# ChristophReich1996/Multi-StyleGAN

Measured on AMD Instinct MI355X. Metric: training images/sec (G+D step, 256^2, seq=3x2ch), higher is better.
Workload: dtype bf16

## Files before the change

multi_stylegan_amd/csrc/conv_wgrad.hip:

```cpp
#include "msg_common.h"
#include <stdlib.h>

typedef __bf16 bf16v8 __attribute__((ext_vector_type(8)));
typedef short s16x4 __attribute__((ext_vector_type(4)));
typedef const __attribute__((address_space(1))) char* gptr_t;
typedef const __attribute__((address_space(1))) u32x4* gvec_t;
typedef __attribute__((address_space(3))) char* lds_t;
__device__ __attribute__((aligned(256))) unsigned int g_wgrad_zero_page[64];

struct WgradParams {
    int B, IH, IW, Cx, I, OH, OW, ldgy, O;
    int OWv, OHv;
    int kh, kw, stride, pad, pixel_shuffle;
    int per_sample, chunks_per_sample, pix_per_chunk, split;
    int xcd_slices;
    int nz;
    int fold;
    int o_tiles, i_tiles, ldgw;
    int oi_major;
    float gain;
    long long gw_zstride;
    long long slab;
};

// ... 392 lines not shown
    float4 t = part[0][lane];
#pragma unroll
    for (int g = 1; g < 4; ++g) { t.x += part[g][lane].x; t.y += part[g][lane].y; t.z += part[g][lane].z; t.w += part[g][lane].w; }
    if (!oi_major) {
        reinterpret_cast<float4*>(out + (long long)n * slab)[v] = t;
        return;
    }
    const int vpr = ldgw >> 2;
    const long long row = v / vpr;
    const int i = (int)(v - row * vpr) * 4;
    const int o = (int)(row / taps), tap = (int)(row - (long long)o * taps);
    float* dst = out + ((long long)n * O + o) * I * taps + (long long)i * taps + tap;
    const float e[4] = {t.x, t.y, t.z, t.w};
#pragma unroll
    for (int k = 0; k < 4; ++k)
        if (i + k < I) dst[(long long)k * taps] = e[k];
}

extern "C" int msg_wgrad_reduce_launch(const float* ws, float* gw, long long slab, int n_out, int chunks, int O, int taps,
                                       int I, int ldgw, int oi_major, void* stream) {
    const long long nvec = slab >> 2;
    const long long blocks = (nvec + 63) / 64;
    if (blocks >= (1ll << 31) || n_out > 65535) return MSG_EUNSUPPORTED;
    hipLaunchKernelGGL(wgrad_reduce_kernel, dim3((unsigned)blocks, (unsigned)n_out), dim3(256), 0, (hipStream_t)stream,
                       ws, gw, slab, chunks, O, taps, I, ldgw, oi_major);
    return MSG_CHECK_LAUNCH();
}

extern "C" int msg_conv2d_wgrad_row3_try(const void* gy, const void* x, float* gw, int dtype,
                                         int B, int IH, int IW, int Cx, int I, int OH, int OW, int ldgy, int O, int ldgw,
                                         int kh, int kw, int stride, int pad, int pixel_shuffle,
                                         int per_sample, int k_chunks, int oi_major, float gain,
                                         float* ws, long long ws_floats, int plan_only, long long* need, void* stream);

static int wgrad_impl(const void* gy, const void* x, float* gw, int dtype,
                      int B, int IH, int IW, int Cx, int I, int OH, int OW, int ldgy, int O, int ldgw,
                      int kh, int kw, int stride, int pad, int pixel_shuffle,
                      int per_sample, int k_chunks, int oi_major, float gain,
                      float* ws, long long ws_floats, int plan_only, long long* need, void* stream) {
    *need = 0;
    if (B == 0) return MSG_OK;
    if (B < 0 || IH <= 0 || IW <= 0 || OH <= 0 || OW <= 0 || O <= 0 || I <= 0 || kh <= 0 ||
        kw <= 0 || stride <= 0 || Cx <= 0 || ldgy <= 0 || ldgw < I || ldgw % 4 || k_chunks <= 0)
        return MSG_EINVAL;
    if (!plan_only && (!gy || !x || !gw)) return MSG_EINVAL;
    const int split = dtype == MSG_F32_SPLIT ? 3 : 0;
    if (split) dtype = MSG_F32;
    if (dtype != MSG_F32 && dtype != MSG_BF16) return MSG_EUNSUPPORTED;
    const int esz = dtype == MSG_BF16 ? 2 : 4, vec = 16 / esz;
    if (Cx % vec || ldgy % vec) return MSG_EUNSUPPORTED;
    if (!plan_only && (((uintptr_t)gy | (uintptr_t)x | (uintptr_t)gw | (uintptr_t)ws) & 15u)) return MSG_EUNSUPPORTED;
    {
        const int r3 = msg_conv2d_wgrad_row3_try(gy, x, gw, dtype, B, IH, IW, Cx, I, OH, OW, ldgy, O, ldgw, kh, kw, stride, pad,
                                                 pixel_shuffle, per_sample, k_chunks, oi_major, gain, ws, ws_floats, plan_only,
                                                 need, stream);
        if (r3 < 0) return r3;
        if (r3) return MSG_OK;
    }
    WgradParams p{};
    p.B = B; p.IH = IH; p.IW = IW; p.Cx = Cx; p.I = I; p.OH = OH; p.OW = OW; p.ldgy = ldgy; p.O = O;
    p.kh = kh; p.kw = kw; p.stride = stride; p.pad = pad; p.pixel_shuffle = pixel_shuffle;
    p.per_sample = per_sample;
    p.chunks_per_sample = k_chunks;
    const int kp = dtype == MSG_BF16 ? 64 : 32;
    static const int variant = msg_tunable("MSG_CONV_VARIANT", 0);
    static const int pad_rows = msg_tunable("MSG_WGRAD_PAD_ROWS", 1);
    const long long gy_bytes = (long long)(pixel_shuffle ? 4 : 1) * OH * OW * ldgy * esz;
    const long long x_bytes = (long long)IH * IW * Cx * esz;
    int owv = OW, ohv = OH;
    if (pad_rows && !pixel_shuffle && !(kp % OW == 0 || OW % kp == 0)) {
        int v = 1;
        while (v < OW) v <<= 1;
        if ((long long)v * 15 <= (long long)OW * 16) {
            owv = v;
            if (v < kp && (OH * v) % kp) ohv = ((OH * v + kp - 1) / kp * kp) / v;
        }
    }
    const bool can_fold0 = !per_sample && variant != 3;
    auto uni_ok = [&](int wl) {
        const long long np = (long long)(wl == OW ? OH : ohv) * wl;
        bool u = variant != 2 && variant != 1 && (kp % wl == 0 || wl % kp == 0) && gy_bytes < (1ll << 31) && x_bytes < (1ll << 31);
        if (can_fold0 && B * np < (1ll << 31) && u &&
            !((np % kp == 0 || kp % np == 0) && B * gy_bytes < 0x7ffffff0ll && B * x_bytes < 0x7ffffff0ll))
            u = false;
        return u;
    };
    bool uni = uni_ok(owv);
    if (!uni && owv != OW) { owv = OW; uni = uni_ok(OW); }
    if (owv == OW) ohv = OH;
    p.OWv = owv;
// ... 93 lines not shown
```

include/msg_hip.h:

```cpp
#ifndef MSG_HIP_H
#define MSG_HIP_H

#ifdef __cplusplus
extern "C" {
#endif

enum { MSG_OK = 0, MSG_EINVAL = -1, MSG_EUNSUPPORTED = -2, MSG_ELAUNCH = -3 };
enum { MSG_F32 = 0, MSG_BF16 = 1, MSG_F16 = 2, MSG_F64 = 3, MSG_F32_SPLIT = 4 };

#define MSG_ABI_VERSION 5
int msg_abi_version(void);
const char* msg_build_arch(void);
const char* msg_strerror(int code);

int msg_upfirdn2d(const void* x, const float* fir, void* y, int dtype,
                  int major, int in_h, int in_w, int minor, int kh, int kw,
                  int up_x, int up_y, int down_x, int down_y,
                  int pad_x0, int pad_x1, int pad_y0, int pad_y1, void* stream);

int msg_upfirdn2d_pitched(const void* x, const float* fir, void* y, int dtype,
                          int major, int in_h, int in_w, int minor, int in_pitch, int kh, int kw,
                          int up_x, int up_y, int down_x, int down_y,
                          int pad_x0, int pad_x1, int pad_y0, int pad_y1, void* stream);

// ... 147 lines not shown
                                  int kh, int kw, int stride, int pad, long long w_batch_stride,
                                  const void* residual, int res_ld,
                                  const unsigned char* sign_mask, int mask_tile_m, int mask_tile_n,
                                  const void* sign_map, int sign_ld, float alpha, float scale,
                                  float* grad_bias, const float* noise, int noise_batch, float* grad_noise_weight,
                                  float* ws, long long ws_floats, void* stream);

int msg_act_pointwise_head(const void* x, const float* bias, const float* w, float* y, int dtype,
                           long long npix, int C, float wscale, float alpha, float scale, void* stream);
long long msg_act_pointwise_head_backward_workspace(long long npix, int C);
int msg_act_pointwise_head_backward(const void* x, const float* bias, const float* w, const float* gy, void* gx,
                                    float* grad_bias_and_w, int dtype, long long npix, int C, float wscale,
                                    float alpha, float scale, float* ws, long long ws_floats, void* stream);

int msg_linear_fprop(const float* x, const float* w, const float* bias, float* y, int M, int N, int K,
                     float gain, float bias_gain, void* stream);
int msg_linear_dgrad(const float* gy, const float* w, float* gx, int M, int N, int K, float gain, void* stream);
int msg_linear_wgrad(const float* gy, const float* x, float* gw, float* gb, int M, int N, int K,
                     float gain, float bias_gain, void* stream);

int msg_linear_grouped_fprop(const float* x, const int* slot, const float* const* w, const float* const* bias, float* y,
                             int G, int M, int N, int K, int L, float gain, float bias_gain, void* stream);
int msg_linear_grouped_dgrad(const float* gy, const float* const* w, float* gx, int G, int M, int N, int K, float gain,
                             void* stream);
int msg_linear_grouped_wgrad(const float* gy, const float* x, const int* slot, float* gw, float* gb, int G, int M, int N,
                             int K, int L, float gain, float bias_gain, void* stream);
int msg_linear_grouped_wgrad_ptrs(const float* gy, const float* x, const int* slot, float* const* gw, float* const* gb, int G,
                                  int M, int N, int K, int L, float gain, float bias_gain, void* stream);

int msg_conv2d_fprop_plan(int dtype, int B, int IH, int IW, int Cx, int Ck, int OH, int OW, int N,
                          int kh, int kw, long long w_batch_stride);
int msg_conv2d_fprop_upconv_eligible(int B, int IH, int IW, int Cx, int Ck, int OH, int OW, int N, int kh, int kw,
                                     int stride, int pad, int in_up, int pixel_shuffle, long long w_batch_stride);
int msg_conv2d_fprop_thin_eligible(int B, int IH, int IW, int Cx, int Ck, int OH, int OW, int N, int ldy, int kh, int kw,
                                   int stride, int pad, int in_up, int pixel_shuffle, int act_mode);

int msg_flat_adam(float* param, const float* grad, float* exp_avg, float* exp_avg_sq, float* ema, long long n,
                  const float* coef, float lr, float beta1, float beta2, float eps, int step, float ema_decay,
                  void* stream);
int msg_flat_ema(float* ema, const float* param, long long n, float decay, void* stream);

#ifdef __cplusplus
}
#endif
#endif
```

multi_stylegan_amd/_lib.py:

```python
import ctypes
import os
import re

import torch

_HERE = os.path.dirname(os.path.abspath(__file__))
LIB_PATH = os.path.join(_HERE, "libmsg_hip" + ("_" + os.environ["MSG_LIB_VARIANT"] if os.environ.get("MSG_LIB_VARIANT") else "")
                        + ".so")
HEADER_PATH = os.path.join(os.path.dirname(_HERE), "include", "msg_hip.h")

MSG_F32, MSG_BF16, MSG_F16, MSG_F64 = 0, 1, 2, 3
ABI_VERSION = 5
_c = ctypes
_P, _I, _L, _F = _c.c_void_p, _c.c_int, _c.c_longlong, _c.c_float

_SIGNATURES = {
    "msg_abi_version": (_I, []),
    "msg_build_arch": (_c.c_char_p, []),
    "msg_strerror": (_c.c_char_p, [_I]),
    "msg_upfirdn2d": (_I, [_P, _P, _P, _I] + [_I] * 14 + [_P]),
    "msg_upfirdn2d_pitched": (_I, [_P, _P, _P, _I] + [_I] * 15 + [_P]),
    "msg_upfirdn2d_pitched2": (_I, [_P, _P, _P, _I] + [_I] * 16 + [_P]),
    "msg_upfirdn2d_separable": (_I, [_P, _P, _P, _P, _I] + [_I] * 10 + [_P]),
    "msg_upfirdn2d_separable_act": (_I, [_P, _P, _P, _P, _I] + [_I] * 10 + [_P, _P, _P, _I, _F, _F, _P]),
# ... 19 lines not shown
    "msg_conv2d_wgrad": (_I, [_P, _P, _P, _I] + [_I] * 18 + [_F, _P, _L, _P]),
    "msg_conv2d_wgrad_workspace": (_L, [_I] * 18),
    "msg_demod_coeff": (_I, [_P, _P, _P, _I, _I, _I, _I, _F, _F, _P]),
    "msg_scale_rows_cols": (_I, [_P, _P, _P, _P, _I, _I, _I, _I, _I, _I, _F, _P]),
    "msg_modulate_weights": (_I, [_P] * 5 + [_I] * 7 + [_F, _F, _P]),
    "msg_modulate_backward": (_I, [_P] * 6 + [_I] * 6 + [_F, _P]),
    "msg_modulate_backward2": (_I, [_P] * 7 + [_I] * 6 + [_F, _P]),
    "msg_scale_rows_cols2": (_I, [_P] * 6 + [_I] * 6 + [_F, _P]),
    "msg_relayout_weight": (_I, [_P, _P, _P, _P, _I] + [_I] * 7 + [_F, _P]),
    "msg_gather_taps": (_I, [_P, _P, _I] + [_I] * 9 + [_P]),
    "msg_fold_taps": (_I, [_P, _P, _P, _I] + [_I] * 10 + [_P]),
    "msg_scaled_add": (_I, [_P, _P, _P, _I, _L, _F, _F, _P]),
    "msg_rgb_skip_merge": (_I, [_P, _I, _I, _P, _P, _P, _P, _I, _I, _I, _I, _P]),
    "msg_rgb_skip_merge_backward": (_I, [_P, _P, _I, _I, _P, _P, _I, _I, _I, _I, _P]),
    "msg_gamma_merge": (_I, [_P, _P, _P, _P, _I, _L, _F, _P]),
    "msg_gamma_merge_backward_workspace": (_L, []),
    "msg_gamma_merge_backward": (_I, [_P, _P, _P, _P, _P, _P, _I, _L, _F, _P, _P]),
    "msg_scaled_add_rows": (_I, [_P, _P, _P, _I, _L, _I, _L, _L, _L, _F, _F, _P]),
    "msg_flat_adam": (_I, [_P, _P, _P, _P, _P, _L, _P, _F, _F, _F, _F, _I, _F, _P]),
    "msg_flat_ema": (_I, [_P, _P, _L, _F, _P]),
    "msg_softmax_rows": (_I, [_P, _P, _I, _L, _I, _P]),
    "msg_softmax_rows_backward": (_I, [_P, _P, _P, _I, _L, _I, _P]),
    "msg_softmax_rows_backward2": (_I, [_P, _P, _P, _P, _P, _I, _L, _I, _P]),
    "msg_nonlocal_attention_supported": (_I, [_I] * 5),
    "msg_nonlocal_attention_fwd": (_I, [_P] * 5 + [_I] * 6 + [_P]),
    "msg_nonlocal_attention_bwd_splits": (_I, [_I] * 3),
    "msg_nonlocal_attention_bwd": (_I, [_P] * 14 + [_I] * 6 + [_P]),
    "msg_affine_warp": (_I, [_P, _P, _P, _F, _P, _P, _P, _I, _F, _F, _I, _I, _I, _I, _I, _I, _I, _P, _P]),
    "msg_minibatch_stddev_workspace": (_L, [_I] * 5),
    "msg_minibatch_stddev": (_I, [_P, _P, _P, _P, _I] + [_I] * 7 + [_F, _P]),
    "msg_minibatch_stddev_backward": (_I, [_P, _P, _P, _P, _I] + [_I] * 8 + [_F, _P]),
    "msg_conv2d_fprop_plan": (_I, [_I] * 11 + [_L]),
    "msg_conv2d_fprop_upconv_eligible": (_I, [_I] * 14 + [_L]),
    "msg_conv2d_fprop_thin_eligible": (_I, [_I] * 16),
    "msg_maxpool2x2_fwd": (_I, [_P, _P, _P, _I, _I, _I, _I, _I, _L, _P]),
    "msg_maxpool2x2_bwd": (_I, [_P, _P, _P, _I, _I, _I, _I, _I, _P]),
    "msg_maxpool2x2_gather": (_I, [_P, _P, _P, _I, _I, _I, _I, _I, _L, _P]),
    "msg_linear_fprop": (_I, [_P, _P, _P, _P, _I, _I, _I, _F, _F, _P]),
    "msg_linear_dgrad": (_I, [_P, _P, _P, _I, _I, _I, _F, _P]),
    "msg_linear_wgrad": (_I, [_P, _P, _P, _P, _I, _I, _I, _F, _F, _P]),
    "msg_linear_grouped_fprop": (_I, [_P, _P, _P, _P, _P, _I, _I, _I, _I, _I, _F, _F, _P]),
    "msg_linear_grouped_dgrad": (_I, [_P, _P, _P, _I, _I, _I, _I, _F, _P]),
    "msg_linear_grouped_wgrad": (_I, [_P, _P, _P, _P, _P, _I, _I, _I, _I, _I, _F, _F, _P]),
    "msg_linear_grouped_wgrad_ptrs": (_I, [_P, _P, _P, _P, _P, _I, _I, _I, _I, _I, _F, _F, _P]),
}


def declared_symbols():
    text = open(HEADER_PATH).read()
    text = re.sub(r"/\*.*?\*/", "", text, flags=re.S)
    return sorted(set(re.findall(r"\b(msg_[a-z0-9_]+)\s*\(", text)))


class MsgHipError(RuntimeError):
    pass


_lib = None


def lib():
    global _lib
    if _lib is None:
        if not os.path.exists(LIB_PATH):
            raise MsgHipError(f"{LIB_PATH} is missing: build it with `python -m multi_stylegan_amd.build` "
                              "(hipcc, --offload-arch=gfx950). There is no CPU fallback.")
# ... 170 lines not shown
```

multi_stylegan_amd/conv_ops.py:

```python
import math
import os
from typing import Optional, Tuple

import torch
from torch.autograd import Function

from . import _lib
from ._autograd import _derive


def _vec(dtype) -> int:
    return 8 if dtype == torch.bfloat16 else 4


def _round_up(n: int, m: int) -> int:
    return (n + m - 1) // m * m


def _padded_nhwc(b, c, h, w, dtype, device):
    cx = _round_up(c, _vec(dtype))
    buf = torch.empty((b, h, w, cx), dtype=dtype, device=device)
    if cx != c:
        buf[..., c:].zero_()
    return buf.permute(0, 3, 1, 2)[:, :c]
# ... 340 lines not shown
    xv, cx = _nhwc_view(x)
    b, _, ih, iw = xv.shape
    oh, ow = out_hw
    if out is not None:
        y, ldy = _nhwc_view(out)
        if y is not out or pixel_shuffle or out.shape != (b, n, oh, ow) or out.dtype != x.dtype or n % _vec(x.dtype):
            raise _lib.MsgHipError(f"conv fprop: destination {tuple(out.shape)} / {out.stride()} for a {(b, n, oh, ow)} result")
    elif pixel_shuffle:
        y, ldy = _alloc_out(b, n // 4, 2 * oh, 2 * ow, x.dtype, dev)
    else:
        y, ldy = _alloc_out(b, n, oh, ow, x.dtype, dev)
    rows_needed = n * (1 if pixel_shuffle else kh * kw) * ck
    if per_sample:
        ws_ = wk.stride() if wk.ndim == 4 else None
        if ws_ is None or wk.shape[0] != b or ws_[0] < rows_needed or ws_[3] != 1 or \
                (wk.shape[2] > 1 and ws_[2] != wk.shape[3]) or (wk.shape[1] > 1 and ws_[1] != wk.shape[2] * wk.shape[3]):
            raise _lib.MsgHipError(f"conv fprop: per-sample weight image {tuple(wk.shape)} for batch {b}, {n} x {kh * kw} x {ck}")
    elif wk.numel() < rows_needed or not wk.is_contiguous():
        raise _lib.MsgHipError(f"conv fprop: weight image {tuple(wk.shape)} smaller than {n} x {kh * kw} x {ck}")
    wstride = wk.stride(0) if per_sample else 0
    if flops is None:
        flops = 2.0 * b * oh * ow * n * kh * kw * c_real / (in_up * in_up)
    key = "conv_fprop"
    if _lib.kernel_clock.enabled:
        plan = _lib.lib().msg_conv2d_fprop_plan(_lib.dtype_code(x), b, ih, iw, cx, ck, oh, ow, n, kh, kw, wstride)
        key = ("conv_fprop_reg", "conv_fprop_dma", "conv_fprop_pp", "conv_fprop_row3", "conv_fprop_row3n",
               "conv_fprop_thin")[plan]
        if plan == 5 and act is not None:
            key = "conv_fprop_reg"
        if x.dtype == torch.bfloat16 and bias is None and act is None and residual is None and \
                _lib.lib().msg_conv2d_fprop_upconv_eligible(b, ih, iw, cx, ck, oh, ow, n, kh, kw, stride, pad, in_up,
                                                           int(pixel_shuffle), wstride):
            key = "conv_fprop_upconv"
        if _CLOCK_SHAPES:
            key += f"|B{b} {ih}x{iw}->{oh}x{ow} {c_real}->{n} {kh}x{kw} s{stride} up{in_up}" \
                   f"{' ps' if pixel_shuffle else ''}{' per-sample' if per_sample else ''}|"
    with _lib.on_device(dev), _lib.kernel_clock.span((key, 'bf16' if x.dtype == torch.bfloat16 else 'f32'), flops):
        if residual is not None:
            assert bias is None and act is None and in_up == 1 and not pixel_shuffle
            rv, res_ld = _nhwc_view(residual[0])
            assert rv.shape == (b, n, oh, ow) and rv.dtype == x.dtype
            code = _lib.lib().msg_conv2d_fprop_residual(
                xv.data_ptr(), wk.data_ptr(), y.data_ptr(), _contraction_code(x, mode), b, ih, iw, cx, ck, oh, ow, n, ldy, kh, kw,
                stride, pad, wstride, rv.data_ptr(), res_ld, float(residual[1]), _lib.stream_of(dev))
        elif act is None:
            code = _lib.lib().msg_conv2d_fprop(
                xv.data_ptr(), wk.data_ptr(), _lib.ptr(bias), y.data_ptr(), _contraction_code(x, mode), b, ih, iw, cx, ck, oh,
                ow, n, ldy, kh, kw, stride, pad, in_up, int(pixel_shuffle), wstride, _lib.stream_of(dev))
        else:
            assert bias is None and in_up == 1 and not pixel_shuffle
            act_bias, noise, noise_w, alpha, scale = act[:5]
            _lib.require_gpu(x, act_bias, noise, noise_w)
            mask = None
            if len(act) > 5 and act[5] is not None and kh == 3 and stride == 1 and pad == 1:
                pkey = (x.dtype, b, ih, iw, cx, ck, oh, ow, n, kh, kw, wstride)
                mplan = _PLAN_CACHE.get(pkey)
                if mplan is None:
                    mplan = _PLAN_CACHE[pkey] = _lib.lib().msg_conv2d_fprop_plan(_lib.dtype_code(x), b, ih, iw, cx, ck, oh, ow,
                                                                                n, kh, kw, wstride)
                if mplan in (3, 4):
                    from .op_static.fused_act import sign_mask_for
                    mask = sign_mask_for(b, n, oh, ow, x.dtype, dev)
                    if mask is not None:
                        act[5].append((mask, 256 if mplan == 3 else 128, 256 if mplan == 3 else 128))
            code = _lib.lib().msg_conv2d_fprop_act_mask(
                xv.data_ptr(), wk.data_ptr(), y.data_ptr(), _contraction_code(x, mode), b, ih, iw, cx, ck, oh, ow, n, ldy, kh, kw,
# ... 1317 lines not shown
```

multi_stylegan_amd/csrc/conv_fprop.hip:

```cpp
#include "msg_common.h"
#include <stdlib.h>

typedef __bf16 bf16v8 __attribute__((ext_vector_type(8)));
typedef const __attribute__((address_space(1))) char* gptr_t;
typedef const __attribute__((address_space(1))) u32x4* gvec_t;
typedef __attribute__((address_space(3))) char* lds_t;

struct ConvParams {
    int B, IH, IW, Cx, Ck, OH, OW, N, ldy;
    int kh, kw, stride, pad, in_up, pixel_shuffle, per_sample;
    long long x_bstride, w_bstride, y_bstride;
    int Mtot, n_chunks, n_iters, m_tiles, n_tiles;
    ActEpilogue act;
};

constexpr int BM = 128, BN = 128, ROWB = 128;
constexpr int STAGE_BYTES = (BM + BN) * ROWB;
__device__ __attribute__((aligned(256))) unsigned int g_zero_page[16384];

__device__ __forceinline__ int swz(int row, int slot) { return row * ROWB + ((slot ^ ((row >> 1) & 7)) << 4); }

template <int SPLIT>
__device__ __forceinline__ void split_park(const u32x4& raw, char* dst) {
    uint2 pl[3];
// ... 369 lines not shown
        for (int pass = 0; pass < NPASS; ++pass) v[pass] = residual_epilogue_apply<T>(v[pass], r[pass], p.act.res_gain);
    }
    T* ybase = y + (p.pixel_shuffle ? nn : n);
    if (n_ok && lim >= VEC) {
#pragma unroll
        for (int pass = 0; pass < NPASS; ++pass)
            if (gp[pass] >= 0) *reinterpret_cast<u32x4*>(ybase + (long long)gp[pass] * p.ldy) = v[pass];
    } else if (n_ok) {
#pragma unroll
        for (int pass = 0; pass < NPASS; ++pass) {
            if (gp[pass] < 0) continue;
            T tmp[VEC];
            *reinterpret_cast<u32x4*>(tmp) = v[pass];
            T* dst = ybase + (long long)gp[pass] * p.ldy;
            for (int e = 0; e < lim; ++e) dst[e] = tmp[e];
        }
    }
}

extern "C" int msg_conv2d_fprop_pp_try(const void* x, const void* w, const float* bias, void* y,
                                       int B, int IH, int IW, int Cx, int Ck, int OH, int OW, int N, int ldy,
                                       int kh, int kw, int stride, int pad, int in_up, int pixel_shuffle,
                                       long long w_batch_stride, const ActEpilogue* act, void* stream);

extern "C" int msg_conv2d_fprop_pp_eligible(int B, int IH, int IW, int Cx, int Ck, int OH, int OW, int N,
                                            int kh, int kw, long long w_batch_stride);
extern "C" int msg_conv2d_fprop_row3_try(const void* x, const void* w, const float* bias, void* y,
                                         int B, int IH, int IW, int Cx, int Ck, int OH, int OW, int N, int ldy,
                                         int kh, int kw, int stride, int pad, int in_up, int pixel_shuffle,
                                         long long w_batch_stride, const ActEpilogue* act, void* stream);

extern "C" int msg_conv2d_fprop_row3_eligible(int B, int IH, int IW, int Cx, int Ck, int OH, int OW, int N,
                                              int kh, int kw, long long w_batch_stride);
extern "C" int msg_conv2d_fprop_upconv_try(const void* x, const void* w, const float* bias, void* y,
                                           int B, int IH, int IW, int Cx, int Ck, int OH, int OW, int N, int ldy,
                                           int kh, int kw, int stride, int pad, int in_up, int pixel_shuffle,
                                           long long w_batch_stride, const ActEpilogue* act, void* stream);
extern "C" int msg_conv2d_fprop_thin_try(const void* x, const void* w, const float* bias, void* y,
                                         int B, int IH, int IW, int Cx, int Ck, int OH, int OW, int N, int ldy,
                                         int kh, int kw, int stride, int pad, int in_up, int pixel_shuffle,
                                         long long w_batch_stride, const ActEpilogue* act, void* stream);
extern "C" int msg_conv2d_fprop_thin_eligible(int B, int IH, int IW, int Cx, int Ck, int OH, int OW, int N, int ldy,
                                              int kh, int kw, int stride, int pad, int in_up, int pixel_shuffle,
                                              int act_mode);

extern "C" int msg_conv2d_fprop_plan(int dtype, int B, int IH, int IW, int Cx, int Ck, int OH, int OW, int N,
                                     int kh, int kw, long long w_batch_stride) {
    if (dtype == MSG_BF16 && msg_conv2d_fprop_thin_eligible(B, IH, IW, Cx, Ck, OH, OW, N, N <= 8 ? 8 : (N + 7) / 8 * 8, kh, kw, 1,
                                                            0, 1, 0, 0))
        return 5;
    if (dtype == MSG_BF16) {
        const int r3 = msg_conv2d_fprop_row3_eligible(B, IH, IW, Cx, Ck, OH, OW, N, kh, kw, w_batch_stride);
        if (r3) return r3 == 1 ? 3 : 4;
    }
    if (dtype == MSG_BF16 && msg_conv2d_fprop_pp_eligible(B, IH, IW, Cx, Ck, OH, OW, N, kh, kw, w_batch_stride)) return 2;
    const int esz = dtype == MSG_BF16 ? 2 : 4;
    const int n_iters = kh * kw * (Ck / (128 / esz));
    static const int variant = msg_tunable("MSG_CONV_VARIANT", 0);
    const bool fits31 = (long long)(w_batch_stride ? 1 : B) * IH * IW * Cx * esz < 0x7ffffff0ll &&
                        (long long)N * kh * kw * Ck * esz < 0x7ffffff0ll;
    return (fits31 && (variant == 1 || (variant == 0 && n_iters >= 8))) ? 1 : 0;
}

static int conv2d_fprop_impl(const void* x, const void* w, const float* bias, void* y, int dtype,
                             int B, int IH, int IW, int Cx, int Ck, int OH, int OW, int N, int ldy,
                             int kh, int kw, int stride, int pad, int in_up, int pixel_shuffle,
// ... 93 lines not shown
    act.enabled = 3; act.alpha = alpha; act.scale = scale;
    act.residual = residual; act.res_ld = res_ld; act.res_gain = 1.f;
    act.mask = const_cast<unsigned char*>(sign_mask); act.mask_tile_m = mask_tile_m; act.mask_tile_n = mask_tile_n;
    act.sign_src = sign_map; act.sign_ld = sign_ld;
    act.noise = has_noise ? noise : nullptr; act.noise_batch = noise_batch;
    act.part_b = grad_bias ? ws : nullptr;
    act.part_n = has_noise ? ws + need_b : nullptr;
    if (!msg_conv2d_fprop_row3_try(x, w, nullptr, y, B, IH, IW, Cx, Ck, OH, OW, N, ldy, kh, kw, stride, pad, 1, 0, w_batch_stride,
                                   &act, stream))
        return MSG_EUNSUPPORTED;
    if (MSG_CHECK_LAUNCH() != MSG_OK) return MSG_ELAUNCH;
    return msg_bias_act_reduce_launch(act.part_b, grad_bias, N, rows, act.part_n, grad_noise_weight, entries, stream);
}

static int conv2d_fprop_impl(const void* x, const void* w, const float* bias, void* y, int dtype,
                             int B, int IH, int IW, int Cx, int Ck, int OH, int OW, int N, int ldy,
                             int kh, int kw, int stride, int pad, int in_up, int pixel_shuffle,
                             long long w_batch_stride, const ActEpilogue& act, void* stream) {
    if (B == 0) return MSG_OK;
    if (!x || !w || !y || B < 0 || IH <= 0 || IW <= 0 || OH <= 0 || OW <= 0 || N <= 0 || kh <= 0 || kw <= 0 ||
        stride <= 0 || in_up <= 0 || Cx <= 0 || Ck <= 0 || ldy <= 0)
        return MSG_EINVAL;
    const int split = dtype == MSG_F32_SPLIT ? 3 : 0;
    if (split) dtype = MSG_F32;
    if (dtype != MSG_F32 && dtype != MSG_BF16) return MSG_EUNSUPPORTED;
    const int esz = dtype == MSG_BF16 ? 2 : 4, vec = 16 / esz, bke = 128 / esz;
    if (Ck % bke || Cx % vec || (((uintptr_t)x | (uintptr_t)w | (uintptr_t)y) & 15u)) return MSG_EUNSUPPORTED;
    if (pixel_shuffle && (N % 4 || (N / 4) % vec || ldy % vec)) return MSG_EUNSUPPORTED;
    if (!pixel_shuffle && ldy % vec) return MSG_EUNSUPPORTED;
    if (in_up > 1 && stride != 1) return MSG_EUNSUPPORTED;
    if (dtype == MSG_BF16 &&
        msg_conv2d_fprop_thin_try(x, w, bias, y, B, IH, IW, Cx, Ck, OH, OW, N, ldy, kh, kw, stride, pad, in_up, pixel_shuffle,
                                  w_batch_stride, &act, stream))
        return MSG_CHECK_LAUNCH();
    if (dtype == MSG_BF16 &&
        msg_conv2d_fprop_upconv_try(x, w, bias, y, B, IH, IW, Cx, Ck, OH, OW, N, ldy, kh, kw, stride, pad, in_up,
                                    pixel_shuffle, w_batch_stride, &act, stream))
        return MSG_CHECK_LAUNCH();
    if (dtype == MSG_BF16 &&
        msg_conv2d_fprop_row3_try(x, w, bias, y, B, IH, IW, Cx, Ck, OH, OW, N, ldy, kh, kw, stride, pad, in_up,
                                  pixel_shuffle, w_batch_stride, &act, stream))
        return MSG_CHECK_LAUNCH();
    if (dtype == MSG_BF16 &&
        msg_conv2d_fprop_pp_try(x, w, bias, y, B, IH, IW, Cx, Ck, OH, OW, N, ldy, kh, kw, stride, pad, in_up,
                                pixel_shuffle, w_batch_stride, &act, stream))
        return MSG_CHECK_LAUNCH();
    ConvParams p{};
    p.B = B; p.IH = IH; p.IW = IW; p.Cx = Cx; p.Ck = Ck; p.OH = OH; p.OW = OW; p.N = N; p.ldy = ldy;
    p.kh = kh; p.kw = kw; p.stride = stride; p.pad = pad; p.in_up = in_up; p.pixel_shuffle = pixel_shuffle;
    p.per_sample = w_batch_stride != 0;
    p.act = act;
    p.x_bstride = (long long)IH * IW * Cx;
    p.w_bstride = w_batch_stride;
    p.y_bstride = pixel_shuffle ? 4ll * OH * OW * ldy : (long long)OH * OW * ldy;
    const long long mtot = p.per_sample ? (long long)OH * OW : (long long)B * OH * OW;
    if (mtot >= (1ll << 31)) return MSG_EUNSUPPORTED;
    p.Mtot = (int)mtot;
    p.n_chunks = Ck / bke;
    p.n_iters = kh * kw * p.n_chunks;
    if ((long long)(p.n_iters + 1) * ROWB + 128 > 65536) return MSG_EUNSUPPORTED;
    p.m_tiles = (int)((mtot + BM - 1) / BM);
    p.n_tiles = (N + BN - 1) / BN;
    const long long blocks = (long long)p.m_tiles * p.n_tiles;
    if (blocks >= (1ll << 31)) return MSG_EUNSUPPORTED;
    dim3 grid((unsigned)blocks, 1, p.per_sample ? B : 1);
    hipStream_t s = (hipStream_t)stream;
// ... 18 lines not shown
```

Baseline: 157.5.

## Add specialized wgrad kernel for 2x2 pixel-shuffle upsample convolutions

Adds a dedicated bf16 weight-gradient kernel for 2x2 kernels with pixel shuffle (upsample layers). Each block handles one dy row-tap and computes both dx taps, sharing one x tile across two gy tiles. It uses a three-stage LDS DMA pipeline, transposed LDS reads and interleaved MFMA scheduling, plus a cost model for split-K chunking followed by a reduce. The aim is to replace the generic wgrad path's less efficient tiling for this shape, at the cost of a large hand-scheduled kernel that needs more maintenance.

Result: no change. 158.1, median of 6 (+0.4%).

```diff
diff --git a/multi_stylegan_amd/csrc/conv_wgrad.hip b/multi_stylegan_amd/csrc/conv_wgrad.hip
--- a/multi_stylegan_amd/csrc/conv_wgrad.hip
+++ b/multi_stylegan_amd/csrc/conv_wgrad.hip
@@ -448,6 +448,12 @@
                                          int kh, int kw, int stride, int pad, int pixel_shuffle,
                                          int per_sample, int k_chunks, int oi_major, float gain,
                                          float* ws, long long ws_floats, int plan_only, long long* need, void* stream);
+
+extern "C" int msg_conv2d_wgrad_up2_try(const void* gy, const void* x, float* gw, int dtype,
+                                        int B, int IH, int IW, int Cx, int I, int OH, int OW, int ldgy, int O, int ldgw,
+                                        int kh, int kw, int stride, int pad, int pixel_shuffle,
+                                        int per_sample, int k_chunks, int oi_major, float gain,
+                                        float* ws, long long ws_floats, int plan_only, long long* need, void* stream);
 
 static int wgrad_impl(const void* gy, const void* x, float* gw, int dtype,
                       int B, int IH, int IW, int Cx, int I, int OH, int OW, int ldgy, int O, int ldgw,
@@ -472,6 +478,11 @@
                                                  need, stream);
         if (r3 < 0) return r3;
         if (r3) return MSG_OK;
+        const int u2 = msg_conv2d_wgrad_up2_try(gy, x, gw, dtype, B, IH, IW, Cx, I, OH, OW, ldgy, O, ldgw, kh, kw, stride, pad,
+                                                pixel_shuffle, per_sample, k_chunks, oi_major, gain, ws, ws_floats, plan_only,
+                                                need, stream);
+        if (u2 < 0) return u2;
+        if (u2) return MSG_OK;
     }
     WgradParams p{};
     p.B = B; p.IH = IH; p.IW = IW; p.Cx = Cx; p.I = I; p.OH = OH; p.OW = OW; p.ldgy = ldgy; p.O = O;
diff --git a/multi_stylegan_amd/csrc/conv_wgrad_up2.hip b/multi_stylegan_amd/csrc/conv_wgrad_up2.hip
--- /dev/null
+++ b/multi_stylegan_amd/csrc/conv_wgrad_up2.hip
@@ -0,0 +1,300 @@
+#include "msg_common.h"
+#include <stdlib.h>
+#include <type_traits>
+
+typedef __bf16 bf16v8 __attribute__((ext_vector_type(8)));
+typedef short s16x4 __attribute__((ext_vector_type(4)));
+typedef short s16x8 __attribute__((ext_vector_type(8)));
+typedef __attribute__((address_space(3))) char* u2_lds_t;
+
+struct Up2Params {
+    int B, H, W, Cx, I, ldgy, O, ldgw;
+    int per_sample, steps_per_chunk, chunks_per_sample, nz, split;
+    int o_tiles, i_tiles, oi_major;
+    int xcd;
+    float gain;
+    long long gw_zstride, slab;
+};
+
+constexpr int U2_ROW = 256;
+constexpr int U2_KP = 64;
+constexpr int U2_TA = 2 * U2_KP * U2_ROW;
+constexpr int U2_TB = U2_KP * U2_ROW;
+constexpr int U2_STAGE = U2_TA + U2_TB;
+constexpr int U2_OOB = (int)0x80000000;
+
+__global__ __launch_bounds__(256, 1) void conv_wgrad_up2s_kernel(const bf16_t* __restrict__ gy, const bf16_t* __restrict__ x,
+                                                                 float* __restrict__ gw, float* __restrict__ ws, Up2Params p) {
+    __shared__ __attribute__((aligned(1024))) char smem[3 * U2_STAGE];
+    const int tid = threadIdx.x, lane = tid & 63, wid = tid >> 6;
+    const int wid_u = __builtin_amdgcn_readfirstlane(wid);
+    const int wm = wid_u >> 1, wn = wid_u & 1;
+    const int tiles = p.o_tiles * p.i_tiles;
+    const int G = tiles * 2;
+    const int bid = p.xcd ? (int)(blockIdx.x & 7) * (int)(gridDim.x >> 3) + (int)(blockIdx.x >> 3) : (int)blockIdx.x;
+    int z = bid / G;
+    const int rem_ = bid - z * G;
+    int dy = rem_ / tiles;
+    int tile = rem_ - dy * tiles;
+    z = __builtin_amdgcn_readfirstlane(z);
+    dy = __builtin_amdgcn_readfirstlane(dy);
+    tile = __builtin_amdgcn_readfirstlane(tile);
+    if (z >= p.nz) return;
+    const int o0 = __builtin_amdgcn_readfirstlane((tile / p.i_tiles) * 128), i0 = __builtin_amdgcn_readfirstlane((tile % p.i_tiles) * 128);
+    const int segs = p.W / U2_KP;
+    const int steps_per_sample = p.H * segs;
+    int b = 0, s0, s1;
+    if (p.per_sample) {
+        b = z / p.chunks_per_sample;
+        const int chunk = z - b * p.chunks_per_sample;
+        s0 = chunk * p.steps_per_chunk;
+        s1 = min(steps_per_sample, s0 + p.steps_per_chunk);
+    } else {
+        s0 = z * p.steps_per_chunk;
+        s1 = min(p.B * steps_per_sample, s0 + p.steps_per_chunk);
+    }
+    b = __builtin_amdgcn_readfirstlane(b);
+    s0 = __builtin_amdgcn_readfirstlane(s0);
+    s1 = __builtin_amdgcn_readfirstlane(s1);
+    const int n_iters = s1 - s0;
+    int b_s = s0 / steps_per_sample;
+    int row_s = (s0 - b_s * steps_per_sample) / segs;
+    int col_s = (s0 - b_s * steps_per_sample - row_s * segs) * U2_KP;
+    b_s = __builtin_amdgcn_readfirstlane(b_s);
+    row_s = __builtin_amdgcn_readfirstlane(row_s);
+    col_s = __builtin_amdgcn_readfirstlane(col_s);
+
+    const int lrow = lane >> 4, chl = ((lane & 15) - 4 * lrow) & 15;
+    const int oc = o0 + chl * 8, ic = i0 + chl * 8;
+    const bool oc_ok = oc + 8 <= p.ldgy, ic_ok = ic + 8 <= p.Cx;
+    const int u_L = p.ldgy * 2, u_C = p.Cx * 2;
+    int voff_gy[8], voff_x[4];
+#pragma unroll
+    for (int j = 0; j < 8; ++j) {
+        const int r = 4 * (wid_u + 4 * j) + lrow;
+        voff_gy[j] = oc_ok ? (2 * (r & 63) + (r >> 6)) * u_L + oc * 2 : U2_OOB;
+    }
+#pragma unroll
+    for (int j = 0; j < 4; ++j) {
+        const int r = 4 * (wid_u + 4 * j) + lrow;
+        voff_x[j] = ic_ok ? r * u_C + ic * 2 : U2_OOB;
+    }
+    const long long sample_gy = 4ll * p.H * p.W * u_L, sample_x = (long long)p.H * p.W * u_C;
+    const char* gbase = (const char*)gy + (p.per_sample ? (long long)b * sample_gy : 0) + (long long)dy * 2 * p.W * u_L;
+    const char* xbase = (const char*)x + (p.per_sample ? (long long)b * sample_x : 0);
+    const msg_desc_t d_gy = msg_make_desc(gbase), d_x = msg_make_desc(xbase);
+    const unsigned lds0 = (unsigned)(unsigned long long)(u2_lds_t)smem;
+
+    f32x4 acc[2][4][4];
+#pragma unroll
+    for (int k = 0; k < 2; ++k)
+#pragma unroll
+        for (int i = 0; i < 4; ++i)
+#pragma unroll
+            for (int j = 0; j < 4; ++j)
+#pragma unroll
+                for (int e = 0; e < 4; ++e) acc[k][i][j][e] = 0.f;
+
+    int so_gy = 0, so_x = 0;
+    auto load_setup = [&]() __attribute__((always_inline)) {
+        const unsigned row = (unsigned)b_s * (unsigned)p.H + (unsigned)row_s;
+        so_gy = (int)(((2u * row) * (2u * (unsigned)p.W) + 2u * (unsigned)col_s) * (unsigned)u_L);
+        so_x = (int)((row * (unsigned)p.W + (unsigned)col_s) * (unsigned)u_C);
+    };
+    auto load_advance = [&]() __attribute__((always_inline)) {
+        col_s += U2_KP;
+        if (col_s == p.W) { col_s = 0; ++row_s; }
+        if (row_s == p.H) { row_s = 0; ++b_s; }
+    };
+    auto dma_piece = [&](int q, int stage, bool live) __attribute__((always_inline)) {
+#if defined(__HIP_DEVICE_COMPILE__)
+        if (q < 8) {
+            msg_dma16(d_gy, lds0 + stage * U2_STAGE + (wid_u + 4 * q) * 1024, live ? voff_gy[q] : U2_OOB, so_gy);
+        } else {
+            const int j = q - 8;
+            msg_dma16(d_x, lds0 + stage * U2_STAGE + U2_TA + (wid_u + 4 * j) * 1024, live ? voff_x[j] : U2_OOB, so_x);
+        }
+#endif
+    };
+    auto dma_all = [&](int stage, bool live) __attribute__((always_inline)) {
+        load_setup();
+#pragma unroll
+        for (int q = 0; q < 12; ++q) dma_piece(q, stage, live);
+        load_advance();
+    };
+    dma_all(0, n_iters > 0);
+    dma_all(1, n_iters > 1);
+    dma_all(2, n_iters > 2);
+
+    const int g4 = lane >> 4, q = (lane >> 2) & 3, pq = lane & 3;
+    int cA[4], cB[4];
+#pragma unroll
+    for (int t = 0; t < 4; ++t) {
+        cA[t] = (8 * g4 + q) * U2_ROW + ((((wm * 64 + t * 16 + 4 * pq) * 2) + (q << 6)) & (U2_ROW - 1));
+        cB[t] = U2_TA + (8 * g4 + q) * U2_ROW + ((((wn * 64 + t * 16 + 4 * pq) * 2) + (q << 6)) & (U2_ROW - 1));
+    }
+    auto frag = [&](const char* stage_base, int c, int rows) __attribute__((always_inline)) {
+        s16x4 part[2];
+#pragma unroll
+        for (int half = 0; half < 2; ++half)
+            part[half] = __builtin_amdgcn_ds_read_tr16_b64_v4i16(
+                (s16x4 __attribute__((address_space(3)))*)(stage_base + c + (rows + 4 * half) * U2_ROW));
+        return __builtin_bit_cast(bf16v8, (s16x8)__builtin_shufflevector(part[0], part[1], 0, 1, 2, 3, 4, 5, 6, 7));
+    };
+    bf16v8 fa[2][2][4], fb[2][4];
+    auto read_nth = [&](int f, int s, const char* base) __attribute__((always_inline)) {
+        if (f == 0) fb[s][0] = frag(base, cB[0], 32 * s);
+        else if (f < 5) fa[s][0][f - 1] = frag(base, cA[f - 1], 32 * s);
+        else if (f < 8) fb[s][f - 4] = frag(base, cB[f - 4], 32 * s);
+        else fa[s][1][f - 8] = frag(base, cA[f - 8], 64 + 32 * s);
+    };
+    auto mfma = [&](int s, int k, int i, int j) __attribute__((always_inline)) {
+        f32x4& c = acc[k][i][j];
+        const bf16v8& af = fa[s][k][i];
+        const bf16v8& bfr = fb[s][j];
+#if defined(__HIP_DEVICE_COMPILE__)
+        asm("v_mfma_f32_16x16x32_bf16 %0, %1, %2, %0" : "+a"(c) : "v"(af), "v"(bfr));
+#endif
+    };
+    asm volatile("s_waitcnt vmcnt(24)" ::: "memory");
+    __syncthreads();
+#pragma unroll
+    for (int f = 0; f < 12; ++f) read_nth(f, 0, smem);
+
+    auto k_step = [&](auto stage_tag, int it) __attribute__((always_inline)) {
+        constexpr int ST = decltype(stage_tag)::value;
+        const char* sa = smem + ST * U2_STAGE;
+        const char* sn = smem + ((ST + 1) % 3) * U2_STAGE;
+        const bool live3 = it + 3 < n_iters;
+#pragma unroll
+        for (int m = 0; m < 32; ++m) {
+            mfma(0, m / 16, (m / 4) % 4, m % 4);
+            if (m < 24 && (m & 1) == 0) read_nth(m / 2, 1, sa);
+            __builtin_amdgcn_sched_barrier(0);
+        }
+        asm volatile("s_waitcnt vmcnt(12) lgkmcnt(0)" ::: "memory");
+        __builtin_amdgcn_sched_barrier(0);
+        asm volatile("s_barrier" ::: "memory");
+        __builtin_amdgcn_sched_barrier(0);
+#pragma unroll
+        for (int m = 0; m < 32; ++m) {
+            mfma(1, m / 16, (m / 4) % 4, m % 4);
+            if (m < 24 && (m & 1) == 0) read_nth(m / 2, 0, sn);
+            if (m == 5) load_setup();
+            if (m >= 7 && (m & 1) == 1 && m < 31) dma_piece((m - 7) / 2, ST, live3);
+            if (m == 31) load_advance();
+            __builtin_amdgcn_sched_barrier(0);
+        }
+    };
+    int it = 0;
+    for (; it + 2 < n_iters; it += 3) {
+        k_step(std::integral_constant<int, 0>{}, it);
+        k_step(std::integral_constant<int, 1>{}, it + 1);
+        k_step(std::integral_constant<int, 2>{}, it + 2);
+    }
+    if (it < n_iters) k_step(std::integral_constant<int, 0>{}, it);
+    if (it + 1 < n_iters) k_step(std::integral_constant<int, 1>{}, it + 1);
+    asm volatile("s_nop 7\n\ts_nop 7\n\ts_nop 7" ::: "memory");
+    asm volatile("s_waitcnt vmcnt(0)" ::: "memory");
+
+    const int l15 = lane & 15;
+    float* gz = p.split ? ws + (long long)z * p.slab : gw + (p.per_sample ? (long long)b * p.gw_zstride : 0);
+    const bool oi_major = p.oi_major && !p.split;
+#pragma unroll
+    for (int k = 0; k < 2; ++k) {
+        const int tap = dy * 2 + k;
+#pragma unroll
+        for (int i = 0; i < 4; ++i)
+#pragma unroll
+            for (int j = 0; j < 4; ++j) {
+                const int icn = i0 + wn * 64 + j * 16 + l15;
+                if (icn >= p.ldgw) continue;
+#pragma unroll
+                for (int e = 0; e < 4; ++e) {
+                    const int o = o0 + wm * 64 + i * 16 + 4 * g4 + e;
+                    if (o >= p.O) continue;
+                    float* dst = oi_major ? gz + ((long long)o * p.I + icn) * 4 + tap
+                                          : gz + ((long long)o * 4 + tap) * p.ldgw + icn;
+                    if (oi_major && icn >= p.I) continue;
+                    *dst = acc[k][i][j][e] * p.gain;
+                }
+            }
+    }
+}
+
+extern "C" int msg_wgrad_reduce_launch(const float* ws, float* gw, long long slab, int n_out, int chunks, int O, int taps,
+                                       int I, int ldgw, int oi_major, void* stream);
+
+extern "C" int msg_conv2d_wgrad_up2_try(const void* gy, const void* x, float* gw, int dtype,
+                                        int B, int IH, int IW, int Cx, int I, int OH, int OW, int ldgy, int O, int ldgw,
+                                        int kh, int kw, int stride, int pad, int pixel_shuffle,
+                                        int per_sample, int k_chunks, int oi_major, float gain,
+                                        float* ws, long long ws_floats, int plan_only, long long* need, void* stream) {
+    static const int enabled = msg_tunable("MSG_WGRAD_UP2", 1);
+    if (!enabled || dtype != MSG_BF16 || !pixel_shuffle || kh != 2 || kw != 2 || OW % U2_KP || IH != OH || IW != OW)
+        return 0;
+    const long long gy_bytes = 4ll * OH * OW * ldgy * 2, x_bytes = (long long)IH * IW * Cx * 2;
+    const long long nb = per_sample ? 1 : B;
+    if (nb * gy_bytes >= 0x7ffffff0ll || nb * x_bytes >= 0x7ffffff0ll) return 0;
+    Up2Params p{};
+    p.B = B; p.H = OH; p.W = OW; p.Cx = Cx; p.I = I; p.ldgy = ldgy; p.O = O; p.ldgw = ldgw;
+    p.per_sample = per_sample;
+    p.o_tiles = (O + 127) / 128;
+    p.i_tiles = (I + 127) / 128;
+    p.oi_major = oi_major;
+    p.gain = gain;
+    p.gw_zstride = oi_major ? (long long)O * I * 4 : (long long)O * 4 * ldgw;
+    p.slab = (long long)O * 4 * ldgw;
+    const long long steps_per_sample = (long long)OH * (OW / U2_KP);
+    const long long tiles = (long long)p.o_tiles * p.i_tiles * 2;
+    long long zs, chunks_per_out;
+    if (per_sample) {
+        if (k_chunks <= 1) {
+            static const int slab_cost_ps = msg_tunable("MSG_WGRAD_UP2_SLAB_COST_PS", 12);
+            long long best = -1;
+            for (long long c = 1; c <= 4 && c * 8 <= steps_per_sample; ++c) {
+                const long long rounds = ((long long)B * tiles * c + 255) / 256;
+                const long long cost = rounds * ((steps_per_sample + c - 1) / c + 3 + (c > 1 ? slab_cost_ps : 0));
+                if (best < 0 || cost < best) { best = cost; k_chunks = (int)c; }
+            }
+            if (best < 0) k_chunks = 1;
+        }
+        p.chunks_per_sample = k_chunks;
+        p.steps_per_chunk = (int)((steps_per_sample + k_chunks - 1) / k_chunks);
+        zs = (long long)B * k_chunks;
+        chunks_per_out = k_chunks;
+    } else {
+        static const int slab_cost = msg_tunable("MSG_WGRAD_UP2_SLAB_COST", 4);
+        const long long steps = (long long)B * steps_per_sample;
+        long long chunks = 1, best = -1;
+        const long long cmax = steps / 4 < 4096 ? steps / 4 : 4096;
+        for (long long c = 1; c <= cmax; ++c) {
+            const long long rounds = (tiles * c + 255) / 256;
+            const long long cost = rounds * ((steps + c - 1) / c + 3 + (c > 1 ? slab_cost : 0));
+            if (best < 0 || cost < best) { best = cost; chunks = c; }
+            if (tiles * c > 4096) break;
+        }
+        p.steps_per_chunk = (int)((steps + chunks - 1) / chunks);
+        zs = (steps + p.steps_per_chunk - 1) / p.steps_per_chunk;
+        p.chunks_per_sample = (int)zs;
+        chunks_per_out = zs;
+    }
+    p.split = chunks_per_out > 1;
+    p.nz = (int)zs;
+    const long long nblk = zs * tiles;
+    if (zs > (1 << 24) || nblk >= (1ll << 31)) return 0;
+    static const int xcd = msg_tunable("MSG_WGRAD_UP2_XCD", 1);
+    p.xcd = xcd && nblk % 8 == 0;
+    *need = p.split ? zs * p.slab : 0;
+    if (plan_only) return 1;
+    if (p.split && (!ws || ws_floats < *need)) return MSG_EINVAL;
+    hipLaunchKernelGGL(conv_wgrad_up2s_kernel, dim3((unsigned)nblk), dim3(256), 0, (hipStream_t)stream,
+                       (const bf16_t*)gy, (const bf16_t*)x, gw, ws, p);
+    if (MSG_CHECK_LAUNCH() != MSG_OK) return MSG_ELAUNCH;
+    if (p.split) {
+        const int rc = msg_wgrad_reduce_launch(ws, gw, p.slab, per_sample ? B : 1, (int)chunks_per_out, O, 4, I, ldgw,
+                                               oi_major, stream);
+        if (rc != MSG_OK) return rc;
+    }
+    return 1;
+}
```

## Add warp-specialized subpixel 1x1 conv kernel for per-sample pixel-shuffle fprop

Applied to the files above, without the earlier changes.

Adds a new bf16 kernel for per-sample-weight 1x1 convolutions with 512 input channels followed by pixel shuffle. It stages the activation tile in LDS once, streams weight slices through a register ring using MFMA, and hands results through an LDS patch to dedicated store waves that write the shuffled output directly. The goal is to overlap GEMM compute with the scattered pixel-shuffle stores and to reuse the activation tile across all N slices. It is tried before the existing upconv and pp paths, is enabled by default, and adds barrier-heavy producer/consumer synchronisation with large LDS use at one block per CU.

New measurement: 157.5 before, 158.1 after (median of 6 runs). About the same (+0.4%).

```diff
diff --git a/include/msg_hip.h b/include/msg_hip.h
--- a/include/msg_hip.h
+++ b/include/msg_hip.h
@@ -203,6 +203,8 @@
                           int kh, int kw, long long w_batch_stride);
 int msg_conv2d_fprop_upconv_eligible(int B, int IH, int IW, int Cx, int Ck, int OH, int OW, int N, int kh, int kw,
                                      int stride, int pad, int in_up, int pixel_shuffle, long long w_batch_stride);
+int msg_conv2d_fprop_subpixel_eligible(int B, int IH, int IW, int Cx, int Ck, int OH, int OW, int N, int kh, int kw,
+                                       int stride, int pad, int in_up, int pixel_shuffle, long long w_batch_stride);
 int msg_conv2d_fprop_thin_eligible(int B, int IH, int IW, int Cx, int Ck, int OH, int OW, int N, int ldy, int kh, int kw,
                                    int stride, int pad, int in_up, int pixel_shuffle, int act_mode);
 
diff --git a/multi_stylegan_amd/_lib.py b/multi_stylegan_amd/_lib.py
--- a/multi_stylegan_amd/_lib.py
+++ b/multi_stylegan_amd/_lib.py
@@ -75,6 +75,7 @@
     "msg_minibatch_stddev_backward": (_I, [_P, _P, _P, _P, _I] + [_I] * 8 + [_F, _P]),
     "msg_conv2d_fprop_plan": (_I, [_I] * 11 + [_L]),
     "msg_conv2d_fprop_upconv_eligible": (_I, [_I] * 14 + [_L]),
+    "msg_conv2d_fprop_subpixel_eligible": (_I, [_I] * 14 + [_L]),
     "msg_conv2d_fprop_thin_eligible": (_I, [_I] * 16),
     "msg_maxpool2x2_fwd": (_I, [_P, _P, _P, _I, _I, _I, _I, _I, _L, _P]),
     "msg_maxpool2x2_bwd": (_I, [_P, _P, _P, _I, _I, _I, _I, _I, _P]),
diff --git a/multi_stylegan_amd/conv_ops.py b/multi_stylegan_amd/conv_ops.py
--- a/multi_stylegan_amd/conv_ops.py
+++ b/multi_stylegan_amd/conv_ops.py
@@ -396,6 +396,10 @@
                 _lib.lib().msg_conv2d_fprop_upconv_eligible(b, ih, iw, cx, ck, oh, ow, n, kh, kw, stride, pad, in_up,
                                                            int(pixel_shuffle), wstride):
             key = "conv_fprop_upconv"
+        if x.dtype == torch.bfloat16 and bias is None and act is None and residual is None and \
+                _lib.lib().msg_conv2d_fprop_subpixel_eligible(b, ih, iw, cx, ck, oh, ow, n, kh, kw, stride, pad, in_up,
+                                                             int(pixel_shuffle), wstride):
+            key = "conv_fprop_subpixel"
         if _CLOCK_SHAPES:
             key += f"|B{b} {ih}x{iw}->{oh}x{ow} {c_real}->{n} {kh}x{kw} s{stride} up{in_up}" \
                    f"{' ps' if pixel_shuffle else ''}{' per-sample' if per_sample else ''}|"
diff --git a/multi_stylegan_amd/csrc/conv_fprop.hip b/multi_stylegan_amd/csrc/conv_fprop.hip
--- a/multi_stylegan_amd/csrc/conv_fprop.hip
+++ b/multi_stylegan_amd/csrc/conv_fprop.hip
@@ -425,6 +425,10 @@
 
 extern "C" int msg_conv2d_fprop_row3_eligible(int B, int IH, int IW, int Cx, int Ck, int OH, int OW, int N,
                                               int kh, int kw, long long w_batch_stride);
+extern "C" int msg_conv2d_fprop_subpixel_try(const void* x, const void* w, const float* bias, void* y,
+                                             int B, int IH, int IW, int Cx, int Ck, int OH, int OW, int N, int ldy,
+                                             int kh, int kw, int stride, int pad, int in_up, int pixel_shuffle,
+                                             long long w_batch_stride, const ActEpilogue* act, void* stream);
 extern "C" int msg_conv2d_fprop_upconv_try(const void* x, const void* w, const float* bias, void* y,
                                            int B, int IH, int IW, int Cx, int Ck, int OH, int OW, int N, int ldy,
                                            int kh, int kw, int stride, int pad, int in_up, int pixel_shuffle,
@@ -584,6 +588,10 @@
     if (dtype == MSG_BF16 &&
         msg_conv2d_fprop_thin_try(x, w, bias, y, B, IH, IW, Cx, Ck, OH, OW, N, ldy, kh, kw, stride, pad, in_up, pixel_shuffle,
                                   w_batch_stride, &act, stream))
+        return MSG_CHECK_LAUNCH();
+    if (dtype == MSG_BF16 &&
+        msg_conv2d_fprop_subpixel_try(x, w, bias, y, B, IH, IW, Cx, Ck, OH, OW, N, ldy, kh, kw, stride, pad, in_up,
+                                      pixel_shuffle, w_batch_stride, &act, stream))
         return MSG_CHECK_LAUNCH();
     if (dtype == MSG_BF16 &&
         msg_conv2d_fprop_upconv_try(x, w, bias, y, B, IH, IW, Cx, Ck, OH, OW, N, ldy, kh, kw, stride, pad, in_up,
diff --git a/multi_stylegan_amd/csrc/conv_subpixel.hip b/multi_stylegan_amd/csrc/conv_subpixel.hip
--- /dev/null
+++ b/multi_stylegan_amd/csrc/conv_subpixel.hip
@@ -0,0 +1,243 @@
+#include "msg_common.h"
+#include <stdlib.h>
+
+typedef __bf16 bf16v8 __attribute__((ext_vector_type(8)));
+typedef const __attribute__((address_space(1))) char* gptr_t;
+typedef __attribute__((address_space(3))) char* lds_t;
+
+struct SubpixelParams {
+    int B, H, W, N, O, ldy;
+    long long x_bstride, w_bstride, y_bstride;
+    int m_tiles, xcd_samples, rotate;
+};
+
+constexpr int SP_M = 128, SP_K = 512, SP_ROW = SP_K * 2;
+constexpr int SP_MW = 4;
+constexpr int SP_HALF = 64 * 64 * 2;
+constexpr int SP_RING = 8;
+
+#ifndef MSG_SUBPIXEL_DIAG
+#define MSG_SUBPIXEL_DIAG 0
+#endif
+#define SP_BARRIER() do { __builtin_amdgcn_sched_barrier(0); asm volatile("s_barrier" ::: "memory"); \
+                          __builtin_amdgcn_sched_barrier(0); } while (0)
+
+template <int KORD>
+__global__ __launch_bounds__(64 * 2 * SP_MW, 1) void conv_subpixel_kernel(const bf16_t* __restrict__ x,
+                                                                           const bf16_t* __restrict__ w,
+                                                                           bf16_t* __restrict__ y, SubpixelParams p) {
+    __shared__ __attribute__((aligned(16))) char smem[SP_M * SP_ROW + SP_MW * SP_HALF];
+    const int tid = threadIdx.x, lane = tid & 63;
+    const int wid_u = __builtin_amdgcn_readfirstlane(tid >> 6);
+    const int lr = lane & 31, lh = lane >> 5;
+    int b, tile;
+    if (p.xcd_samples) {
+        const int xcd = blockIdx.x & 7, k = blockIdx.x >> 3;
+        const int j = k / p.m_tiles;
+        tile = k - j * p.m_tiles;
+        b = xcd + 8 * j;
+    } else {
+        b = blockIdx.x / p.m_tiles;
+        tile = blockIdx.x - b * p.m_tiles;
+    }
+    b = __builtin_amdgcn_readfirstlane(b);
+    tile = __builtin_amdgcn_readfirstlane(tile);
+    const int m0 = tile * SP_M;
+    const int hw = p.H * p.W;
+
+    {
+        const gptr_t xb = (gptr_t)(x + (long long)b * p.x_bstride);
+#pragma unroll 4
+        for (int j = 0; j < SP_M / (2 * SP_MW); ++j) {
+            const int r = wid_u * (SP_M / (2 * SP_MW)) + j;
+            const int m = m0 + r < hw ? m0 + r : 0;
+            const gptr_t src = xb + ((long long)m * SP_K + ((lane ^ (r & 15)) << 3)) * 2;
+            __builtin_amdgcn_global_load_lds(src, (lds_t)(smem + r * SP_ROW), 16, 0, 0);
+        }
+        asm volatile("s_waitcnt vmcnt(0)" ::: "memory");
+        __syncthreads();
+    }
+
+    const int n_rounds = p.N / (64 * SP_MW);
+    const int rot = p.rotate ? tile % n_rounds : 0;
+    auto slice_n0 = [&](int s, int wv) __attribute__((always_inline)) {
+        const int sl = s + rot < n_rounds ? s + rot : s + rot - n_rounds;
+        return (sl * SP_MW + wv) * 64;
+    };
+    if (wid_u < SP_MW) {
+        const bf16_t* wb = w + (long long)b * p.w_bstride;
+        char* patch = smem + SP_M * SP_ROW + wid_u * SP_HALF;
+        const int swz = lr & 15;
+        const int k_lane = KORD == 0 ? 32 * lh : 8 * lh;
+        auto k_step = [](int st) { return KORD == 0 ? 64 * (st >> 2) + 8 * (st & 3) : 64 * (st >> 2) + 16 * (st & 3); };
+        bf16v8 fb[SP_RING][2];
+        auto load_w = [&](int n0, int st) __attribute__((always_inline)) {
+#pragma unroll
+            for (int j = 0; j < 2; ++j)
+                fb[st % SP_RING][j] = *reinterpret_cast<const bf16v8*>(wb + (long long)(n0 + 32 * j + lr) * SP_K + k_lane + k_step(st));
+        };
+        bf16v8 fa[4];
+        unsigned abase = (unsigned)(lr * SP_ROW) + ((unsigned)((k_lane >> 3) ^ swz) << 4);
+        auto read_a = [&](int st, int i) __attribute__((always_inline)) {
+            const unsigned off = abase ^ ((unsigned)(k_step(st) >> 3) << 4);
+            fa[i] = *reinterpret_cast<const bf16v8*>(smem + off + 32 * i * SP_ROW);
+        };
+#pragma unroll
+        for (int st = 0; st < 4; ++st) load_w(slice_n0(0, wid_u), st);
+        for (int s = 0; s < n_rounds; ++s) {
+            const int n0 = slice_n0(s, wid_u);
+            const int n0_next = s + 1 < n_rounds ? slice_n0(s + 1, wid_u) : n0;
+            asm volatile("" : "+v"(abase));
+            f32x16 acc[4][2];
+#pragma unroll
+            for (int i = 0; i < 4; ++i)
+#pragma unroll
+                for (int j = 0; j < 2; ++j)
+#pragma unroll
+                    for (int e = 0; e < 16; ++e) acc[i][j][e] = 0.f;
+#pragma unroll
+            for (int i = 0; i < 4; ++i) read_a(0, i);
+#if MSG_SUBPIXEL_DIAG == 2
+            if (false)
+#endif
+#pragma unroll
+            for (int st = 0; st < SP_K / 16; ++st) {
+                if (st % 4 == 0) {
+#pragma unroll
+                    for (int a = 4; a < 8; ++a) {
+                        const int ahead = st + a;
+                        if (ahead < SP_K / 16) load_w(n0, ahead);
+                        else if (s + 1 < n_rounds) load_w(n0_next, ahead - SP_K / 16);
+                    }
+                    __builtin_amdgcn_sched_barrier(0);
+                }
+#pragma unroll
+                for (int i = 0; i < 4; ++i) {
+#pragma unroll
+                    for (int j = 0; j < 2; ++j)
+                        acc[i][j] = __builtin_amdgcn_mfma_f32_32x32x16_bf16(fb[st % SP_RING][j], fa[i], acc[i][j], 0, 0, 0);
+                    if (st + 1 < SP_K / 16) read_a(st + 1, i);
+                }
+            }
+            if (s > 0) SP_BARRIER();
+#pragma unroll
+            for (int hf = 0; hf < 2; ++hf) {
+#pragma unroll
+                for (int ii = 0; ii < 2; ++ii) {
+                    const int i = 2 * hf + ii;
+#pragma unroll
+                    for (int j = 0; j < 2; ++j)
+#pragma unroll
+                        for (int g = 0; g < 4; ++g) {
+                            const int unit = 8 * j + 2 * g + lh;
+                            constexpr float z = KORD == 0 ? -0.f : 0.f;
+                            uint2 pk;
+                            pk.x = (unsigned)f2bf(acc[i][j][4 * g + 0] + z) | ((unsigned)f2bf(acc[i][j][4 * g + 1] + z) << 16);
+                            pk.y = (unsigned)f2bf(acc[i][j][4 * g + 2] + z) | ((unsigned)f2bf(acc[i][j][4 * g + 3] + z) << 16);
+                            *reinterpret_cast<uint2*>(patch + ii * (SP_HALF / 2) + lr * 128 + ((unit ^ (lr & 15)) << 3)) = pk;
+                        }
+                }
+                asm volatile("s_waitcnt lgkmcnt(0)" ::: "memory");
+                SP_BARRIER();
+                if (hf == 0) SP_BARRIER();
+            }
+        }
+        SP_BARRIER();
+    } else {
+        const int sw = wid_u - SP_MW;
+        const char* patch = smem + SP_M * SP_ROW + sw * SP_HALF;
+        bf16_t* yb = y + (long long)b * p.y_bstride;
+        const int er = lane >> 3, ec = lane & 7;
+        int opix[16];
+#pragma unroll
+        for (int k = 0; k < 16; ++k) {
+            const int m = m0 + 8 * k + er;
+            const int oh = m / p.W, ow = m - oh * p.W;
+            opix[k] = m < hw ? 2 * oh * (2 * p.W) + 2 * ow : -1;
+        }
+        u32x4 v[16];
+        auto read_half = [&](int hf) __attribute__((always_inline)) {
+#pragma unroll
+            for (int ii = 0; ii < 2; ++ii)
+#pragma unroll
+                for (int pass = 0; pass < 4; ++pass) {
+                    const int row = pass * 8 + er;
+                    u32x4 t = *reinterpret_cast<const u32x4*>(patch + ii * (SP_HALF / 2) + row * 128 + ((ec ^ ((row & 15) >> 1)) << 4));
+                    if (row & 1) t = u32x4{t[2], t[3], t[0], t[1]};
+                    v[8 * hf + 4 * ii + pass] = t;
+                }
+            asm volatile("s_waitcnt lgkmcnt(0)" ::: "memory");
+        };
+        for (int s = 0; s < n_rounds; ++s) {
+            const int n0 = slice_n0(s, sw);
+            const int q = n0 / p.O, c0 = n0 - q * p.O;
+            const long long qoff = (long long)(q >> 1) * (2 * p.W) + (q & 1);
+            if (s > 0) SP_BARRIER();
+            SP_BARRIER();
+            read_half(0);
+            SP_BARRIER();
+            SP_BARRIER();
+            read_half(1);
+            bf16_t* yc = yb + c0 + ec * 8;
+#pragma unroll
+            for (int k = 0; k < 16; ++k)
+                if (opix[k] >= 0 && MSG_SUBPIXEL_DIAG != 1)
+                    *reinterpret_cast<u32x4*>(yc + ((long long)opix[k] + qoff) * p.ldy) = v[k];
+        }
+        SP_BARRIER();
+    }
+}
+
+extern "C" int msg_conv2d_fprop_upconv_eligible(int B, int IH, int IW, int Cx, int Ck, int OH, int OW, int N, int kh, int kw,
+                                                int stride, int pad, int in_up, int pixel_shuffle, long long w_batch_stride);
+extern "C" int msg_conv2d_fprop_pp_eligible(int B, int IH, int IW, int Cx, int Ck, int OH, int OW, int N,
+                                            int kh, int kw, long long w_batch_stride);
+
+static int subpixel_order(int B, int IH, int IW, int Cx, int Ck, int OH, int OW, int N, int kh, int kw, int stride, int pad,
+                          int in_up, int pixel_shuffle, long long w_batch_stride) {
+    static const int enabled = msg_tunable("MSG_CONV_SUBPIXEL", 1);
+    if (!enabled || !pixel_shuffle || w_batch_stride == 0 || kh != 1 || kw != 1 || stride != 1 || pad != 0 || in_up != 1)
+        return -1;
+    if (Cx != SP_K || Ck != SP_K || N < 256 || N % (64 * SP_MW) || IH != OH || IW != OW) return -1;
+    if (w_batch_stride < (long long)N * SP_K) return -1;
+    const long long hw = (long long)OH * OW;
+    if (hw < 4096 || hw >= (1ll << 30)) return -1;
+    const long long blocks = ((hw + SP_M - 1) / SP_M) * B;
+    if (blocks < 256 || blocks >= (1ll << 31)) return -1;
+    if (msg_conv2d_fprop_upconv_eligible(B, IH, IW, Cx, Ck, OH, OW, N, kh, kw, stride, pad, in_up, pixel_shuffle, w_batch_stride))
+        return 0;
+    if (msg_conv2d_fprop_pp_eligible(B, IH, IW, Cx, Ck, OH, OW, N, kh, kw, w_batch_stride)) return 1;
+    return -1;
+}
+
+extern "C" int msg_conv2d_fprop_subpixel_eligible(int B, int IH, int IW, int Cx, int Ck, int OH, int OW, int N, int kh, int kw,
+                                                  int stride, int pad, int in_up, int pixel_shuffle, long long w_batch_stride) {
+    return subpixel_order(B, IH, IW, Cx, Ck, OH, OW, N, kh, kw, stride, pad, in_up, pixel_shuffle, w_batch_stride) >= 0;
+}
+
+extern "C" int msg_conv2d_fprop_subpixel_try(const void* x, const void* w, const float* bias, void* y,
+                                             int B, int IH, int IW, int Cx, int Ck, int OH, int OW, int N, int ldy,
+                                             int kh, int kw, int stride, int pad, int in_up, int pixel_shuffle,
+                                             long long w_batch_stride, const ActEpilogue* act, void* stream) {
+    if (bias || (act && act->enabled)) return 0;
+    const int order = subpixel_order(B, IH, IW, Cx, Ck, OH, OW, N, kh, kw, stride, pad, in_up, pixel_shuffle, w_batch_stride);
+    if (order < 0) return 0;
+    SubpixelParams p{};
+    p.B = B; p.H = OH; p.W = OW; p.N = N; p.O = N / 4; p.ldy = ldy;
+    p.x_bstride = (long long)IH * IW * Cx;
+    p.w_bstride = w_batch_stride;
+    p.y_bstride = 4ll * OH * OW * ldy;
+    p.m_tiles = (int)(((long long)OH * OW + SP_M - 1) / SP_M);
+    static const int xcd_order = msg_tunable("MSG_UPCONV_XCD", 1);
+    p.xcd_samples = xcd_order && B % 8 == 0;
+    static const int rotate = msg_tunable("MSG_SUBPIXEL_ROT", 1);
+    p.rotate = rotate;
+    dim3 grid((unsigned)((long long)p.m_tiles * B));
+    if (order == 0)
+        hipLaunchKernelGGL(conv_subpixel_kernel<0>, grid, dim3(64 * 2 * SP_MW), 0, (hipStream_t)stream, (const bf16_t*)x,
+                           (const bf16_t*)w, (bf16_t*)y, p);
+    else
+        hipLaunchKernelGGL(conv_subpixel_kernel<1>, grid, dim3(64 * 2 * SP_MW), 0, (hipStream_t)stream, (const bf16_t*)x,
+                           (const bf16_t*)w, (bf16_t*)y, p);
+    return 1;
+}
```
